# Deeptanshu-sankhwar/horizonml

Measured on AMD Instinct MI355X. Metric: images/sec, higher is better.
Workload: dtype bf16; 1 GPU; model=resnet18_cifar10, global_batch=64, image=3x32x32, parallelism=dp1, optimizer=adam, exec=graph, comm=none

## Files before the change

horizonml_amd/engine/flat.py:

```python
from __future__ import annotations

from typing import List

import torch
import torch.nn as nn

from .. import ops as _ops
from ..models.layers import ConvBNAct, DepthwiseConvBNAct, Linear


class FlatParamManager:
    def __init__(self, model: nn.Module, device: torch.device):
        _ops.extension().set_wgrad_defer(True)
        params = [p for p in model.parameters() if p.requires_grad]
        total = sum(p.numel() for p in params)
        self.params = params
        self.numel = total
        self.master = torch.zeros(total, device=device)
        self.grad = torch.zeros(total, device=device)
        self.shadow = torch.zeros(total, device=device, dtype=torch.bfloat16)
        self.slices = {}
        off = 0
        for p in params:
            n = p.numel()
            with torch.no_grad():
                self.master[off:off + n].copy_(p.data.flatten())
            p.data = self.master[off:off + n].view(p.shape)
            p.grad = self.grad[off:off + n].view(p.shape)
            self.slices[id(p)] = (off, n)
            off += n
        with torch.no_grad():
            self.shadow.copy_(self.master)

        convs = []
        for m in model.modules():
            if isinstance(m, (ConvBNAct, Linear, DepthwiseConvBNAct)):
                woff, wn = self.slices[id(m.weight)]
                m.weight_bf16 = self.shadow[woff:woff + wn].view(
                    m.weight.shape)
                m._managed = True
                if isinstance(m, ConvBNAct):
                    convs.append((m, woff, wn))
        stats_total = sum(2 * m.out_ch for m, _, _ in convs)
        self.stats_arena = torch.zeros(max(1, stats_total), device=device)
        soff = 0
        for m, _, _ in convs:
            m._stats_buf = self.stats_arena[soff:soff + 2 * m.out_ch]
            soff += 2 * m.out_ch

        rsck_total = sum(wn for _, _, wn in convs)
        self.rsck = torch.zeros(rsck_total, device=device,
                                dtype=torch.bfloat16)
        meta: List[List[int]] = []
        doff = 0
        self.max_elem = 1
        for m, woff, wn in convs:
            K, R, S, C = m.weight.shape
            meta.append([woff, doff, wn, (K << 16) | C])
            m._w_rsck = self.rsck[doff:doff + wn].view(R, S, C, K)
            doff += wn
            self.max_elem = max(self.max_elem, wn)
        self.meta = (torch.tensor(meta, dtype=torch.int32, device=device)
                     if meta else None)
        self.refresh_rsck()

    def refresh_rsck(self):
        if self.meta is not None:
            _ops.extension().permute_krsc_rsck(self.shadow, self.rsck,
                                               self.meta, self.max_elem)

    def zero_grad(self):
        self.grad.zero_()


def _sched_buffers(schedule, dev):
    if schedule is None:
        return None, None
    return schedule.table().to(dev), torch.zeros(1, device=dev)


class HorizonAdam:

# ... 122 lines not shown
```

horizonml_amd/models/_functional_gpu.py:

```python
from __future__ import annotations

import torch

from .. import ops as _ops


def _C():
    return _ops.extension()


def _bwd_done(mod):
    cb = getattr(mod, "_bwd_done_cb", None)
    if cb is not None:
        cb()


def _cl(t: torch.Tensor) -> torch.Tensor:
    if t.dim() == 4 and not t.is_contiguous(memory_format=torch.channels_last):
        return t.contiguous(memory_format=torch.channels_last)
    if t.dim() != 4 and not t.is_contiguous():
        return t.contiguous()
    return t


class ConvBNActFn(torch.autograd.Function):
    @staticmethod
    def forward(ctx, x, weight, bn_weight, bn_bias, residual, mod):
        x = _cl(x)
        w_bf16 = mod._shadow()
        if residual is not None:
            residual = _cl(residual)
        stats_buf = (getattr(mod, "_stats_buf", None)
                     if mod.training else None)
        y, convout, smean, sinvstd = _C().conv_bn_act_fwd(
            x, w_bf16, bn_weight, bn_bias, mod.running_mean, mod.running_var,
            mod.stride, mod.padding, mod.momentum, mod.eps, mod.training,
            mod.act, residual, stats_buf)
        ctx.save_for_backward(x, y, convout, w_bf16, bn_weight, bn_bias,
                              smean, sinvstd)
        ctx.mod = mod
        ctx.has_res = residual is not None
        return y

    @staticmethod
    def backward(ctx, dy):
        x, y, convout, w_bf16, gamma, beta, smean, sinvstd = \
            ctx.saved_tensors
        mod = ctx.mod
        need_dx = ctx.needs_input_grad[0]
        w_rsck = getattr(mod, "_w_rsck", None)
        if need_dx and (w_rsck is None or w_rsck.numel() != w_bf16.numel()):
            w_rsck = w_bf16.permute(1, 2, 3, 0).contiguous()
        dy = _cl(dy.to(torch.bfloat16) if dy.dtype != torch.bfloat16 else dy)
        direct = (getattr(mod, "_managed", False)
                  and mod.weight.grad is not None)
        dw_out = mod.weight.grad if direct else None
        dg_out = mod.bn_weight.grad if direct else None
        db_out = mod.bn_bias.grad if direct else None
        dx, dw, dgamma, dbeta, dres = _C().conv_bn_act_bwd(
            dy, y, x, w_bf16, w_rsck if need_dx else w_bf16, convout, gamma,
            beta, smean, sinvstd, mod.stride, mod.padding, mod.act, need_dx,
            ctx.has_res, dw_out, dg_out, db_out, None, None, 0, False, None,
            None)
        _bwd_done(mod)
        if direct:
            return (dx if need_dx else None, None, None, None,
                    dres if ctx.has_res else None, None)
        return (dx if need_dx else None, dw, dgamma, dbeta,
                dres if ctx.has_res else None, None)


def conv_bn_act(x, mod, residual=None):
    return ConvBNActFn.apply(x, mod.weight, mod.bn_weight, mod.bn_bias,
                             residual, mod)


class DwConvBNActFn(torch.autograd.Function):
    @staticmethod
    def forward(ctx, x, weight, bn_weight, bn_bias, residual, mod):
        x = _cl(x)
        w_bf16 = mod._shadow()
        if residual is not None:
            residual = _cl(residual)
        y, convout, smean, sinvstd = _C().dw_conv_bn_fwd(
            x, w_bf16, bn_weight, bn_bias, mod.running_mean,
            mod.running_var, mod.stride, mod.padding, mod.momentum, mod.eps,
            mod.training, mod.act, residual)
        ctx.save_for_backward(x, y, convout, w_bf16, bn_weight, bn_bias,
                              smean, sinvstd)
        ctx.mod = mod
        ctx.has_res = residual is not None
        return y

# ... 86 lines not shown


def linear(x, mod):
    return LinearFn.apply(x, mod.weight, mod.bias, mod)


class CrossEntropyFn(torch.autograd.Function):
    @staticmethod
    def forward(ctx, logits, target, label_smoothing=0.0):
        logits = logits.float().contiguous()
        if label_smoothing == 0.0:
            loss, dlogits = _C().cross_entropy_fwd_bwd(logits, target)
        else:
            loss, dlogits = _C().cross_entropy_ls_fwd_bwd(
                logits, target, float(label_smoothing))
        ctx.save_for_backward(dlogits)
        return loss

    @staticmethod
    def backward(ctx, gout):
        (dlogits,) = ctx.saved_tensors
        return dlogits * gout, None, None


def cross_entropy(logits: torch.Tensor, target: torch.Tensor,
                  label_smoothing: float = 0.0) -> torch.Tensor:
    if logits.is_cuda:
        return CrossEntropyFn.apply(logits, target, float(label_smoothing))
    return torch.nn.functional.cross_entropy(
        logits.float(), target, label_smoothing=float(label_smoothing))


def _rsck(mod, w_bf16):
    w = getattr(mod, "_w_rsck", None)
    if w is None or w.numel() != w_bf16.numel():
        w = w_bf16.permute(1, 2, 3, 0).contiguous()
    return w


class ResBlockFn(torch.autograd.Function):

    @staticmethod
    def forward(ctx, x, mods, ds_mod, *params):
        x = _cl(x)
        training = mods[0].training
        if ds_mod is not None:
            y_ds, convout_ds, smean_ds, sinvstd_ds = _C().conv_bn_act_fwd(
                x, ds_mod._shadow(), ds_mod.bn_weight, ds_mod.bn_bias,
                ds_mod.running_mean, ds_mod.running_var, ds_mod.stride,
                ds_mod.padding, ds_mod.momentum, ds_mod.eps, training,
                ds_mod.act, None,
                getattr(ds_mod, "_stats_buf", None) if training else None)
            identity = y_ds
        else:
            identity = x
        h = x
        saved = [x]
        n = len(mods)
        for i, m in enumerate(mods):
            res = identity if i == n - 1 else None
            y, convout, smean, sinvstd = _C().conv_bn_act_fwd(
                h, m._shadow(), m.bn_weight, m.bn_bias, m.running_mean,
                m.running_var, m.stride, m.padding, m.momentum, m.eps,
                training, m.act, res,
                getattr(m, "_stats_buf", None) if training else None)
            saved += [y, convout, smean, sinvstd, m._shadow(),
# ... 95 lines not shown
```

horizonml_amd/ops/csrc/bind.cpp:

```cpp
#include <torch/extension.h>
#include <c10/hip/HIPStream.h>
#include <c10/hip/HIPCachingAllocator.h>

#include <memory>
#include <vector>

#include "launch.h"

namespace {

using torch::Tensor;

hipStream_t cur_stream() { return c10::hip::getCurrentHIPStream().stream(); }

bool g_deterministic = false;
void set_deterministic(bool on) {
  g_deterministic = on;
  set_kernels_deterministic(on ? 1 : 0);
}
bool deterministic_enabled() { return g_deterministic; }

void set_bn_owner(bool on) { set_kernels_bn_owner(on ? 1 : 0); }
bool bn_owner_enabled() { return kernels_bn_owner() != 0; }
std::vector<int64_t> bn_owner_launches() {
  long f = 0, b = 0;
  bn_owner_launch_counts(&f, &b);
  return {(int64_t)f, (int64_t)b};
}

struct PendingWgrad {
  torch::Tensor x, dconv, dw;
  ConvP p;
};

bool g_wgrad_defer = false;
std::vector<PendingWgrad> g_pending;
torch::Tensor g_wgrad_ws;

void set_wgrad_defer(bool on) { g_wgrad_defer = on; }
bool wgrad_defer_enabled() { return g_wgrad_defer; }
int64_t wgrad_pending() { return (int64_t)g_pending.size(); }

static inline int cdiv_i(long a, long b) { return (int)((a + b - 1) / b); }

void flush_one_group(int lo, int hi);

void flush_wgrad() {
  if (g_pending.empty()) return;
  const int total = (int)g_pending.size();
  int lo = 0;
  while (lo < total) {
    std::vector<const void*> seen;
    int hi = lo;
    for (; hi < total; hi++) {
      const void* ptr = g_pending[hi].dw.data_ptr();
      bool dup = false;
      for (const void* q : seen)
        if (q == ptr) { dup = true; break; }
      if (dup) break;
      seen.push_back(ptr);
    }
// ... 225 lines not shown
                          (int)act, splitk, own, st);
      return {y, convout, smean, sinvstd};
    }
    if (training)
      launch_stats_reduce(ws.data_ptr<float>(), stats_ptr, (long)p.M, K,
                          splitk, st);
    launch_bn_apply_f32(ws.data_ptr<float>(), res_ptr, y.data_ptr(),
                        convout.data_ptr(), stats_ptr,
                        gamma.data_ptr<float>(), beta.data_ptr<float>(),
                        running_mean.data_ptr<float>(),
                        running_var.data_ptr<float>(),
                        training ? smean.data_ptr<float>() : nullptr,
                        training ? sinvstd.data_ptr<float>() : nullptr,
                        (long)p.M, K, (float)momentum, (float)eps,
                        training ? 1 : 0, (int)act, splitk, st);
  } else {
    launch_conv_fwd(x.data_ptr(), w.data_ptr(), convout.data_ptr(),
                    g_deterministic ? nullptr : stats_ptr, p, st);
    if (g_deterministic && training)
      launch_stats_bf16_det(convout.data_ptr(), stats_ptr, (long)p.M, K,
                            st);
    launch_bn_apply(convout.data_ptr(), res_ptr, y.data_ptr(), stats_ptr,
                    gamma.data_ptr<float>(), beta.data_ptr<float>(),
                    running_mean.data_ptr<float>(),
                    running_var.data_ptr<float>(),
                    training ? smean.data_ptr<float>() : nullptr,
                    training ? sinvstd.data_ptr<float>() : nullptr,
                    (long)p.M, K, (float)momentum, (float)eps,
                    training ? 1 : 0, (int)act, st);
  }
  return {y, convout, smean, sinvstd};
}

std::vector<Tensor> conv_bn_act_bwd(
    Tensor dy, Tensor y, Tensor x, Tensor w, Tensor w_rsck, Tensor convout,
    Tensor gamma, Tensor beta, Tensor save_mean, Tensor save_invstd,
    int64_t stride, int64_t pad, int64_t act, bool need_dx, bool has_res,
    c10::optional<Tensor> dw_out, c10::optional<Tensor> dgamma_out,
    c10::optional<Tensor> dbeta_out, c10::optional<Tensor> dx_accum,
    c10::optional<std::vector<Tensor>> fuse_up, int64_t up_mask_mode,
    bool sums_ready, c10::optional<Tensor> sum_dz_in,
    c10::optional<Tensor> sum_dzx_in) {
  check_cl(dy, "dy");
  check_cl(y, "y");
  check_cl(x, "x");
  check_cl(convout, "convout");
  int K = (int)w.size(0), R = (int)w.size(1), S = (int)w.size(2);
  ConvP p = make_convp(x, K, R, S, (int)stride, (int)pad);
  auto fopt = x.options().dtype(torch::kFloat32);
  auto st = cur_stream();

  bool direct = dw_out.has_value();
  int mask_mode = act == 1 ? (has_res ? 1 : 2)
                 : act == 2 ? (has_res ? 3 : 4) : 0;
  Tensor sum_dz, sum_dzx;
  const int own = sums_ready ? 0 : bn_owner_bwd_pick((long)p.M, K, 0);
  if (sums_ready) {
    sum_dz = direct ? *dbeta_out : *sum_dz_in;
    sum_dzx = direct ? *dgamma_out : *sum_dzx_in;
  } else {
    sum_dz = direct ? *dbeta_out : at::zeros({K}, fopt);
    sum_dzx = direct ? *dgamma_out : at::zeros({K}, fopt);
    if (!own)
      launch_bnact_bwd_reduce(dy.data_ptr(), y.data_ptr(),
                              convout.data_ptr(),
                              save_mean.data_ptr<float>(),
                              save_invstd.data_ptr<float>(),
                              gamma.data_ptr<float>(),
// ... 17 lines not shown
                        gamma.data_ptr<float>(), beta.data_ptr<float>(),
                        sum_dz.data_ptr<float>(), sum_dzx.data_ptr<float>(),
                        dconv.data_ptr(), dres_ptr, (long)p.M, K, mask_mode,
                        own, st);
  else
    launch_bn_bwd_apply(dy.data_ptr(), y.data_ptr(), convout.data_ptr(),
                        save_mean.data_ptr<float>(),
                        save_invstd.data_ptr<float>(),
                        gamma.data_ptr<float>(), beta.data_ptr<float>(),
                        sum_dz.data_ptr<float>(), sum_dzx.data_ptr<float>(),
                        dconv.data_ptr(), dres_ptr, (long)p.M, K, mask_mode,
                        st);

  Tensor dw = direct ? *dw_out
                     : at::zeros({(int64_t)K, R, S, (int64_t)p.C}, fopt);
  if (direct && g_wgrad_defer) {
    g_pending.push_back({x, dconv, dw, p});
  } else {
    int msplit = wgrad_msplit(p);
    Tensor ws;
    float* ws_ptr = nullptr;
    if (msplit > 1) {
      ws = at::empty({(long)msplit * K * p.Kd}, fopt);
      ws_ptr = ws.data_ptr<float>();
    }
    launch_wgrad(x.data_ptr(), dconv.data_ptr(), dw.data_ptr<float>(), ws_ptr,
                 p, st);
  }

  TORCH_CHECK(need_dx || !fuse_up.has_value(),
              "fuse_up requires need_dx (the fused reduce rides the dx "
              "production)");
  Tensor dx;
  if (need_dx) {
    TORCH_CHECK(w_rsck.is_contiguous() &&
                    w_rsck.scalar_type() == torch::kBFloat16,
                "w_rsck must be contiguous bf16");
    int accum = dx_accum.has_value() ? 1 : 0;
    dx = accum ? *dx_accum : empty_cl_bf16(p.Nb, p.C, p.H, p.W, x);
    ConvP pd = p;
    pd.M = p.Nb * p.H * p.W;
    pd.Kd = R * S * K;
    int splitk = conv_dgrad_splitk(p);
    const bool fuse = fuse_up.has_value();
    if (splitk > 1) {
      int kchunk = ((pd.Kd + splitk - 1) / splitk + 31) / 32 * 32;
      splitk = (pd.Kd + kchunk - 1) / kchunk;
      Tensor wsd = at::empty({(long)splitk * pd.M * p.C}, fopt);
      launch_conv_dgrad(dconv.data_ptr(), w_rsck.data_ptr(), nullptr,
                        wsd.data_ptr<float>(), splitk, pd, 0, st);
      if (fuse) {
        auto& f = *fuse_up;
        launch_cast_bnact(wsd.data_ptr<float>(), dx.data_ptr(), (long)pd.M,
                          p.C, splitk, accum, f[0].data_ptr(),
                          f[1].defined() ? f[1].data_ptr() : f[0].data_ptr(),
                          f[2].data_ptr<float>(), f[3].data_ptr<float>(),
                          f[4].data_ptr<float>(), f[5].data_ptr<float>(),
                          f[6].data_ptr<float>(), f[7].data_ptr<float>(),
                          (int)up_mask_mode, st);
      } else {
        launch_cast_f32_bf16(wsd.data_ptr<float>(), dx.data_ptr(),
                             (long)pd.M * p.C, splitk, accum, st);
      }
    } else {
      launch_conv_dgrad(dconv.data_ptr(), w_rsck.data_ptr(), dx.data_ptr(),
                        nullptr, 1, pd, accum, st);
      if (fuse) {
        auto& f = *fuse_up;
        launch_bnact_bwd_reduce(dx.data_ptr(), f[1].defined()
                                    ? f[1].data_ptr() : f[0].data_ptr(),
                                f[0].data_ptr(), f[2].data_ptr<float>(),
                                f[3].data_ptr<float>(),
                                f[4].data_ptr<float>(),
                                f[5].data_ptr<float>(),
                                f[6].data_ptr<float>(),
                                f[7].data_ptr<float>(), (long)pd.M, p.C,
                                (int)up_mask_mode, st);
      }
    }
  }
  return {dx, dw, sum_dzx, sum_dz, dres};
}

void check_dw_geometry(int R, int S, int64_t stride, int H, int W,
                       int64_t pad) {
  TORCH_CHECK(R >= 1 && S >= 1 && R * S <= 25,
              "depthwise filter must have R*S <= 25 taps, got ", R, "x", S);
  TORCH_CHECK(stride >= 1, "depthwise stride must be >= 1, got ", stride);
  TORCH_CHECK(pad >= 0, "depthwise pad must be >= 0, got ", pad);
  TORCH_CHECK(H + 2 * pad >= R && W + 2 * pad >= S,
              "depthwise output must be at least 1x1: input ", H, "x", W,
              ", pad ", pad, ", filter ", R, "x", S);
}

std::vector<Tensor> dw_conv_bn_fwd(
    Tensor x, Tensor w, Tensor gamma, Tensor beta, Tensor running_mean,
    Tensor running_var, int64_t stride, int64_t pad, double momentum,
    double eps, bool training, int64_t act, c10::optional<Tensor> residual) {
  check_cl(x, "x");
  TORCH_CHECK(w.is_cuda() && w.scalar_type() == torch::kBFloat16 &&
                  w.is_contiguous() && w.dim() == 3,
              "w must be contiguous bf16 [R,S,C]");
  int Nb = (int)x.size(0), C = (int)x.size(1), H = (int)x.size(2),
      W = (int)x.size(3);
  int R = (int)w.size(0), S = (int)w.size(1);
  TORCH_CHECK((int)w.size(2) == C, "depthwise channel mismatch");
  check_dw_geometry(R, S, stride, H, W, pad);
  int Ho = (H + 2 * (int)pad - R) / (int)stride + 1;
  int Wo = (W + 2 * (int)pad - S) / (int)stride + 1;
  long M = (long)Nb * Ho * Wo;
  auto fopt = x.options().dtype(torch::kFloat32);
  Tensor convout = empty_cl_bf16(Nb, C, Ho, Wo, x);
  Tensor y = empty_cl_bf16(Nb, C, Ho, Wo, x);
// ... 555 lines not shown
        py::arg("wd"), py::arg("decoupled"), py::arg("zero_grad"),
        py::arg("extra_zero") = py::none(), py::arg("grad_bf16") = py::none(),
        py::arg("grad_scale") = 1.0, py::arg("probe_prev") = py::none(),
        py::arg("probe_sumsq") = py::none(),
        py::arg("probe_out") = py::none());
  m.def("sgd_step_sched", &sgd_step_sched, py::arg("master"),
        py::arg("grad"), py::arg("mom"), py::arg("shadow"), py::arg("step_t"),
        py::arg("lr_table"), py::arg("lr_out"), py::arg("lr"), py::arg("mu"),
        py::arg("wd"), py::arg("nesterov"), py::arg("zero_grad"),
        py::arg("grad_bf16") = py::none(), py::arg("grad_scale") = 1.0,
        py::arg("probe_prev") = py::none(),
        py::arg("probe_sumsq") = py::none(),
        py::arg("probe_out") = py::none());
  m.def("permute_krsc_rsck", &permute_krsc_rsck);
  m.def("grad_divergence", &grad_divergence);
  m.def("normalize_u8", &normalize_u8);
  m.def("augment_normalize_u8", &augment_normalize_u8, py::arg("x"),
        py::arg("state"), py::arg("mean"), py::arg("std"), py::arg("pad"),
        py::arg("flip"), py::arg("params") = py::none());
  m.def("bn_reduce_bench", &bn_reduce_bench);
  m.def("bn_fwd_pair_bench", &bn_fwd_pair_bench);
  m.def("bn_bwd_pair_bench", &bn_bwd_pair_bench);
  m.def("set_bn_owner", &set_bn_owner);
  m.def("bn_owner_enabled", &bn_owner_enabled);
  m.def("bn_owner_launches", &bn_owner_launches);
  m.def("set_deterministic", &set_deterministic);
  m.def("deterministic_enabled", &deterministic_enabled);
  m.def("set_wgrad_defer", &set_wgrad_defer);
  m.def("wgrad_defer_enabled", &wgrad_defer_enabled);
  m.def("wgrad_pending", &wgrad_pending);
  m.def("flush_wgrad", &flush_wgrad);
  m.def("flush_wgrad_range", &flush_wgrad_range);
  m.def("wgrad_only", &wgrad_only);
}
```

horizonml_amd/ops/csrc/conv_kernels.hip:

```cpp
#include "common.h"

template <int MODE>
DEV int a_addr(const ConvP& p, const MagicP& mg, int m, int k, bool& valid) {
  if (MODE == 0) {
    valid = (m < p.M) & (k < p.Kd);
    return m * p.Kd + k;
  } else if (MODE == 1) {
    unsigned n = fdiv(m, mg, 0), hw = fmod(m, n, mg, 0);
    unsigned ho = fdiv(hw, mg, 1), wo = fmod(hw, ho, mg, 1);
    unsigned r = fdiv(k, mg, 2), rm = fmod(k, r, mg, 2);
    unsigned sx = fdiv(rm, mg, 3), c = fmod(rm, sx, mg, 3);
    int hi = (int)ho * p.str - p.pad + (int)r;
    int wi = (int)wo * p.str - p.pad + (int)sx;
    valid = (m < p.M) & (k < p.Kd) & (hi >= 0) & (hi < p.H) & (wi >= 0) & (wi < p.W);
    return (((int)n * p.H + hi) * p.W + wi) * p.C + (int)c;
  } else {
    unsigned n = fdiv(m, mg, 0), hw = fmod(m, n, mg, 0);
    unsigned hi = fdiv(hw, mg, 1), wi = fmod(hw, hi, mg, 1);
    unsigned r = fdiv(k, mg, 2), rm = fmod(k, r, mg, 2);
    unsigned sx = fdiv(rm, mg, 3), ko = fmod(rm, sx, mg, 3);
    int hs = (int)hi + p.pad - (int)r, ws = (int)wi + p.pad - (int)sx;
    bool ok = (m < p.M) & (k < p.Kd) & (hs >= 0) & (ws >= 0) &&
              (hs % p.str == 0) && (ws % p.str == 0);
    int ho = hs / p.str, wo = ws / p.str;
// ... 48 lines not shown
          ++hi;
        }
      }
    }
  } else {
    for (int e = 0; e < 8; e++) {
      bool ok;
      int a = a_addr<MODE>(p, mg, m, k + e, ok);
      v.e[e] = ok ? src[a] : (bf16)0.f;
    }
  }
  return v;
}

template <int MODE, bool VEC>
DEV V8 load8_b(const bf16* __restrict__ src, const ConvP& p,
               const MagicP& mg, int n, int k, int Ntot) {
  V8 v;
  if (VEC) {
    bool ok;
    int a = b_addr<MODE>(p, mg, n, k, Ntot, ok);
    if (ok) v.u = *(const uint4*)(src + a);
    else v.u = uint4{0, 0, 0, 0};
  } else {
    for (int e = 0; e < 8; e++) {
      bool ok;
      int a = b_addr<MODE>(p, mg, n, k + e, Ntot, ok);
      v.e[e] = ok ? src[a] : (bf16)0.f;
    }
  }
  return v;
}

#define LDA 40

template <int MODE, bool VECA, bool VECB, bool STATS, bool SPLIT,
          int TM = 64, int TN = 64>
__global__ __launch_bounds__(256) void k_conv_mfma(
    const bf16* __restrict__ A, const bf16* __restrict__ Bw,
    bf16* __restrict__ Y, float* __restrict__ ws_out,
    float* __restrict__ stats, ConvP p, MagicP mg, int Ntot, int kchunk,
    int accum) {
  constexpr int AC = TM / 64;
  constexpr int BC = TN / 64;
  constexpr int MI = TM / 32;
  constexpr int NI = TN / 32;
  constexpr int WM = TM / 2, WN = TN / 2;
  __shared__ bf16 As[2][TM * LDA];
  __shared__ bf16 Bs[2][TN * LDA];

  const int m0 = blockIdx.y * TM, n0 = blockIdx.x * TN;
  const int kbeg = SPLIT ? blockIdx.z * kchunk : 0;
  const int kend = SPLIT ? min(p.Kd, kbeg + kchunk) : p.Kd;
  const int tid = threadIdx.x;
  const int srow = tid >> 2, scol = (tid & 3) * 8;
  const int lane = tid & 63, wave = tid >> 6;
  const int wr = wave >> 1, wc = wave & 1;
  const int fr = lane & 15, fk = lane >> 4;

  f32x4 acc[MI][NI] = {};

#pragma unroll
  for (int j = 0; j < AC; j++) {
    V8 a0 = load8_a<MODE, VECA>(A, p, mg, m0 + j * 64 + srow, kbeg + scol);
    *(V8*)&As[0][(j * 64 + srow) * LDA + scol] = a0;
  }
#pragma unroll
  for (int j = 0; j < BC; j++) {
    V8 b0 = load8_b<MODE, VECB>(Bw, p, mg, n0 + j * 64 + srow, kbeg + scol,
                                Ntot);
    *(V8*)&Bs[0][(j * 64 + srow) * LDA + scol] = b0;
  }
  V8 a_nx[AC], b_nx[BC];
  if (kbeg + 32 < kend) {
#pragma unroll
    for (int j = 0; j < AC; j++)
      a_nx[j] = load8_a<MODE, VECA>(A, p, mg, m0 + j * 64 + srow,
                                    kbeg + 32 + scol);
#pragma unroll
    for (int j = 0; j < BC; j++)
      b_nx[j] = load8_b<MODE, VECB>(Bw, p, mg, n0 + j * 64 + srow,
                                    kbeg + 32 + scol, Ntot);
  }
  __syncthreads();

  int buf = 0;
  for (int k0 = kbeg; k0 < kend; k0 += 32) {
    if (k0 + 32 < kend) {
#pragma unroll
      for (int j = 0; j < AC; j++)
        *(V8*)&As[buf ^ 1][(j * 64 + srow) * LDA + scol] = a_nx[j];
#pragma unroll
      for (int j = 0; j < BC; j++)
        *(V8*)&Bs[buf ^ 1][(j * 64 + srow) * LDA + scol] = b_nx[j];
      if (k0 + 64 < kend) {
#pragma unroll
        for (int j = 0; j < AC; j++)
          a_nx[j] = load8_a<MODE, VECA>(A, p, mg, m0 + j * 64 + srow,
                                        k0 + 64 + scol);
#pragma unroll
        for (int j = 0; j < BC; j++)
          b_nx[j] = load8_b<MODE, VECB>(Bw, p, mg, n0 + j * 64 + srow,
                                        k0 + 64 + scol, Ntot);
      }
    }
    bf16x8 af[MI], bf[NI];
#pragma unroll
    for (int mi = 0; mi < MI; mi++)
      af[mi] =
          *(const bf16x8*)&As[buf][(wr * WM + mi * 16 + fr) * LDA + fk * 8];
#pragma unroll
    for (int ni = 0; ni < NI; ni++)
      bf[ni] =
          *(const bf16x8*)&Bs[buf][(wc * WN + ni * 16 + fr) * LDA + fk * 8];
#pragma unroll
    for (int mi = 0; mi < MI; mi++)
#pragma unroll
      for (int ni = 0; ni < NI; ni++)
        acc[mi][ni] = __builtin_amdgcn_mfma_f32_16x16x32_bf16(
            af[mi], bf[ni], acc[mi][ni], 0, 0, 0);
    buf ^= 1;
    __syncthreads();
  }

  float ssum[NI], ssq[NI];
#pragma unroll
  for (int ni = 0; ni < NI; ni++) ssum[ni] = ssq[ni] = 0.f;
#pragma unroll
  for (int mi = 0; mi < MI; mi++) {
#pragma unroll
    for (int ni = 0; ni < NI; ni++) {
      int gn = n0 + wc * WN + ni * 16 + fr;
#pragma unroll
      for (int q = 0; q < 4; q++) {
        int gm = m0 + wr * WM + mi * 16 + fk * 4 + q;
        if (gm < p.M && gn < Ntot) {
          float v = acc[mi][ni][q];
          if (SPLIT) {
            ws_out[(long)blockIdx.z * p.M * Ntot + (long)gm * Ntot + gn] = v;
          } else {
            long yi = (long)gm * Ntot + gn;
            if (accum) v += b2f(Y[yi]);
            Y[yi] = f2b(v);
            if (STATS) {
              ssum[ni] += v;
              ssq[ni] += v * v;
            }
// ... 487 lines not shown
    if (vec && s) CASE_T(true, true, true, TM, TN);                    \
    else if (vec) CASE_T(true, true, false, TM, TN);                   \
    else if (s) CASE_T(false, false, true, TM, TN);                    \
    else CASE_T(false, false, false, TM, TN);                          \
  } while (0)
  if (tile == 3) DISPATCH(256, 64);
  else if (tile == 2) DISPATCH(128, 128);
  else if (tile == 1) DISPATCH(128, 64);
  else DISPATCH(64, 64);
#undef DISPATCH
#undef CASE_T
}

extern "C" void launch_conv_fwd_splitk(const void* x, const void* w,
                                       float* ws, ConvP p, int splitk,
                                       hipStream_t st) {
  int kchunk = cdiv_h(cdiv_h(p.Kd, splitk), 32) * 32;
  splitk = cdiv_h(p.Kd, kchunk);
  bool vec = (p.C % 8) == 0 && (p.Kd % 8) == 0;
  auto A = (const bf16*)x;
  auto B = (const bf16*)w;
  MagicP mg = make_magic(p, 1);
  int tile = pick_tile(p.M, p.K);
#define SK_T(VA, VB, TM, TN)                                              k_conv_mfma<1, VA, VB, false, true, TM, TN><<<grid, 256, 0, st>>>(          A, B, nullptr, ws, nullptr, p, mg, p.K, kchunk, 0)
#define DISPATCH(TM, TN)                                                  do {                                                                      dim3 grid(cdiv_h(p.K, TN), cdiv_h(p.M, TM), splitk);                    if (vec) SK_T(true, true, TM, TN);                                      else SK_T(false, false, TM, TN);                                      } while (0)
  if (tile == 3) DISPATCH(256, 64);
  else if (tile == 2) DISPATCH(128, 128);
  else if (tile == 1) DISPATCH(128, 64);
  else DISPATCH(64, 64);
#undef DISPATCH
#undef SK_T
}

extern "C" void launch_conv_dgrad(const void* dz, const void* w_rsck,
                                  void* dx, float* ws, int splitk, ConvP p,
                                  int accum, hipStream_t st) {
  bool vec = (p.K % 8) == 0;
  auto A = (const bf16*)dz;
  auto B = (const bf16*)w_rsck;
  if (splitk > 1) {
    int kchunk = cdiv_h(cdiv_h(p.Kd, splitk), 32) * 32;
    splitk = cdiv_h(p.Kd, kchunk);
    MagicP mg = make_magic(p, 2);
    int tile = pick_tile_dgrad(p.M, p.C);
#define SKD_T(VA, VB, TM, TN)                                             k_conv_mfma<2, VA, VB, false, true, TM, TN><<<grid, 256, 0, st>>>(          A, B, nullptr, ws, nullptr, p, mg, p.C, kchunk, 0)
#define DISPATCH(TM, TN)                                                  do {                                                                      dim3 grid(cdiv_h(p.C, TN), cdiv_h(p.M, TM), splitk);                    if (vec) SKD_T(true, true, TM, TN);                                     else SKD_T(false, false, TM, TN);                                     } while (0)
    if (tile == 3) DISPATCH(256, 64);
    else if (tile == 2) DISPATCH(128, 128);
    else if (tile == 1) DISPATCH(128, 64);
    else DISPATCH(64, 64);
#undef DISPATCH
#undef SKD_T
  } else {
    MagicP mg = make_magic(p, 2);
    int tile = pick_tile_dgrad(p.M, p.C);
#define DGRAD_T(VA, VB, TM, TN)                                         \
  k_conv_mfma<2, VA, VB, false, false, TM, TN><<<grid, 256, 0, st>>>(   \
      A, B, (bf16*)dx, nullptr, nullptr, p, mg, p.C, 0, accum)
#define DISPATCH(TM, TN)                                                \
  do {                                                                  \
    dim3 grid(cdiv_h(p.C, TN), cdiv_h(p.M, TM));                        \
    if (vec) DGRAD_T(true, true, TM, TN);                               \
    else DGRAD_T(false, false, TM, TN);                                 \
  } while (0)
    if (tile == 3) DISPATCH(256, 64);
    else if (tile == 2) DISPATCH(128, 128);
    else if (tile == 1) DISPATCH(128, 64);
    else DISPATCH(64, 64);
#undef DISPATCH
#undef DGRAD_T
  }
}
// ... 66 lines not shown
```

horizonml_amd/ops/csrc/launch.h:

```cpp
#pragma once
#include <hip/hip_runtime_api.h>

#include <cstdlib>
#include <type_traits>

struct ConvP {
  int Nb, H, W, C, K;
  int Ho, Wo, R, S;
  int str, pad;
  int M, Kd;
};

struct MagicP {
  unsigned m[4];
  int s[4];
  unsigned d[4];
};

constexpr int WG_MAX_TASKS = 20;

struct WgradTask {
  const void* X;
  const void* Dz;
  float* out;
  ConvP p;
  MagicP mg;
  int Ntot, mchunk, msplit, tx, ty;
  int base;
  int vec;
};

struct WgradBatchArgs {
  int n;
  WgradTask t[WG_MAX_TASKS];
};

struct WredTask {
  const float* ws;
  float* dW;
  long n;
  int msplit;
  int base;
};

struct WredBatchArgs {
  int n;
  WredTask t[WG_MAX_TASKS];
};

static_assert(sizeof(WgradBatchArgs) <= 4096 && sizeof(WredBatchArgs) <= 4096,
              "batched wgrad task tables must fit the kernarg segment");
static_assert(std::is_trivially_copyable_v<WgradBatchArgs> &&
                  std::is_trivially_copyable_v<WredBatchArgs>,
              "batched wgrad task tables are copied into the kernarg segment");

inline void magic_u32(unsigned d, unsigned* m, int* sh) {
  if (d <= 1) { *m = 0; *sh = 0; return; }
  int p = 0;
  while ((1ull << p) < d) p++;
  *m = (unsigned)((((unsigned long long)((1ull << p) - d) << 32) / d) + 1);
  *sh = p;
}

inline MagicP make_magic(const ConvP& p, int mode) {
  MagicP mg{};
  unsigned d[4];
  if (mode == 2) {
    d[0] = (unsigned)(p.H * p.W);
    d[1] = (unsigned)p.W;
    d[2] = (unsigned)(p.S * p.K);
    d[3] = (unsigned)p.K;
  } else {
    d[0] = (unsigned)(p.Ho * p.Wo);
    d[1] = (unsigned)p.Wo;
    d[2] = (unsigned)(p.S * p.C);
    d[3] = (unsigned)p.C;
  }
  for (int i = 0; i < 4; i++) {
    mg.d[i] = d[i] ? d[i] : 1;
    magic_u32(mg.d[i], &mg.m[i], &mg.s[i]);
  }
  return mg;
}

inline long env_long(const char* name, long dflt) {
  const char* e = getenv(name);
  return e ? atol(e) : dflt;
}

extern "C" {

int conv_fwd_splitk(ConvP p);
int conv_dgrad_splitk(ConvP p);
void launch_conv_fwd(const void* x, const void* w, void* y, float* stats,
                     ConvP p, hipStream_t st);
void launch_conv_fwd_splitk(const void* x, const void* w, float* ws, ConvP p,
                            int splitk, hipStream_t st);
void launch_conv_dgrad(const void* dz, const void* w_rsck, void* dx,
                       float* ws, int splitk, ConvP p, int accum,
                       hipStream_t st);
void launch_gemm_bf16(const void* a, const void* b, void* c, int M, int N,
                      int K, hipStream_t st);
int wgrad_msplit(ConvP p);
void launch_wgrad(const void* x, const void* dz, float* dw, float* ws,
                  ConvP p, hipStream_t st);
void launch_wgrad_batched_t(const WgradBatchArgs* args, int blocks, int tk3,
                            int tko, hipStream_t st);
void launch_wgrad_reduce_batched(const WredBatchArgs* args, int blocks,
                                 hipStream_t st);

void set_kernels_deterministic(int on);
void set_kernels_bn_owner(int on);
int kernels_bn_owner();
void bn_owner_launch_counts(long* fwd, long* bwd);
int bn_owner_fwd_pick(long M, int C, int lpr_req);
int bn_owner_bwd_pick(long M, int C, int lpr_req);

void launch_bn_apply(const void* x, const void* res, void* y,
                     const float* stats, const float* gamma,
                     const float* beta, float* rmean, float* rvar,
                     float* smean, float* sinvstd, long M, int C,
                     float momentum, float eps, int training, int act,
                     hipStream_t st);
void launch_bn_apply_f32(const float* ws, const void* res, void* y,
                         void* convout, const float* stats,
                         const float* gamma, const float* beta, float* rmean,
                         float* rvar, float* smean, float* sinvstd, long M,
                         int C, float momentum, float eps, int training,
                         int act, int nsplit, hipStream_t st);
void launch_stats_reduce(const float* ws, float* stats, long M, int C,
                         int nsplit, hipStream_t st);
void launch_stats_bf16_det(const void* x, float* stats, long M, int C,
// ... 100 lines not shown
```

Baseline: 64130 images/sec.

## Read KRSC weights directly in dgrad via LDS transpose reads, drop RSCK copy

Adds a KRSC variant of the MFMA dgrad kernel that loads weights in their native KRSC layout, stores them into LDS with a swizzled offset, and uses ds_read_tr16 transpose reads to build the B fragments. This removes the per-step permute_krsc_rsck kernel after each optimizer step and the separate RSCK weight buffer. It is enabled by default through HZ_DGRAD_KRSC. The dgrad main loop now does strided global loads along K plus transpose LDS reads, which could be slower than the old contiguous loads.

```diff
diff --git a/horizonml_amd/engine/flat.py b/horizonml_amd/engine/flat.py
--- a/horizonml_amd/engine/flat.py
+++ b/horizonml_amd/engine/flat.py
@@ -48,6 +48,14 @@
             m._stats_buf = self.stats_arena[soff:soff + 2 * m.out_ch]
             soff += 2 * m.out_ch
 
+        self.meta = None
+        self.max_elem = 1
+        if _ops.extension().dgrad_krsc_enabled():
+            self.rsck = torch.zeros(0, device=device, dtype=torch.bfloat16)
+            for m, _, _ in convs:
+                if hasattr(m, "_w_rsck"):
+                    del m._w_rsck
+            return
         rsck_total = sum(wn for _, _, wn in convs)
         self.rsck = torch.zeros(rsck_total, device=device,
                                 dtype=torch.bfloat16)
diff --git a/horizonml_amd/models/_functional_gpu.py b/horizonml_amd/models/_functional_gpu.py
--- a/horizonml_amd/models/_functional_gpu.py
+++ b/horizonml_amd/models/_functional_gpu.py
@@ -48,9 +48,7 @@
             ctx.saved_tensors
         mod = ctx.mod
         need_dx = ctx.needs_input_grad[0]
-        w_rsck = getattr(mod, "_w_rsck", None)
-        if need_dx and (w_rsck is None or w_rsck.numel() != w_bf16.numel()):
-            w_rsck = w_bf16.permute(1, 2, 3, 0).contiguous()
+        w_rsck = _rsck(mod, w_bf16) if need_dx else None
         dy = _cl(dy.to(torch.bfloat16) if dy.dtype != torch.bfloat16 else dy)
         direct = (getattr(mod, "_managed", False)
                   and mod.weight.grad is not None)
@@ -58,7 +56,7 @@
         dg_out = mod.bn_weight.grad if direct else None
         db_out = mod.bn_bias.grad if direct else None
         dx, dw, dgamma, dbeta, dres = _C().conv_bn_act_bwd(
-            dy, y, x, w_bf16, w_rsck if need_dx else w_bf16, convout, gamma,
+            dy, y, x, w_bf16, w_rsck, convout, gamma,
             beta, smean, sinvstd, mod.stride, mod.padding, mod.act, need_dx,
             ctx.has_res, dw_out, dg_out, db_out, None, None, 0, False, None,
             None)
@@ -211,6 +209,8 @@
 
 
 def _rsck(mod, w_bf16):
+    if _C().dgrad_krsc_enabled():
+        return None
     w = getattr(mod, "_w_rsck", None)
     if w is None or w.numel() != w_bf16.numel():
         w = w_bf16.permute(1, 2, 3, 0).contiguous()
diff --git a/horizonml_amd/ops/csrc/bind.cpp b/horizonml_amd/ops/csrc/bind.cpp
--- a/horizonml_amd/ops/csrc/bind.cpp
+++ b/horizonml_amd/ops/csrc/bind.cpp
@@ -27,6 +27,10 @@
   bn_owner_launch_counts(&f, &b);
   return {(int64_t)f, (int64_t)b};
 }
+
+bool g_dgrad_krsc = env_long("HZ_DGRAD_KRSC", 1) != 0;
+void set_dgrad_krsc(bool on) { g_dgrad_krsc = on; }
+bool dgrad_krsc_enabled() { return g_dgrad_krsc; }
 
 struct PendingWgrad {
   torch::Tensor x, dconv, dw;
@@ -318,8 +322,101 @@
   return {y, convout, smean, sinvstd};
 }
 
+Tensor dgrad_dx(const Tensor& dconv, const Tensor& w,
+                const c10::optional<Tensor>& w_rsck, const ConvP& p,
+                const c10::optional<Tensor>& dx_accum,
+                const c10::optional<std::vector<Tensor>>& fuse_up,
+                int up_mask_mode, hipStream_t st) {
+  const bool krsc =
+      !w_rsck.has_value() || w_rsck->data_ptr() == w.data_ptr();
+  const Tensor& wt = krsc ? w : *w_rsck;
+  TORCH_CHECK(wt.is_contiguous() && wt.scalar_type() == torch::kBFloat16,
+              krsc ? "w must be contiguous bf16"
+                   : "w_rsck must be contiguous bf16");
+  TORCH_CHECK(wt.numel() == (int64_t)p.K * p.R * p.S * p.C,
+              "dgrad weight has ", wt.numel(), " elements, expected K*R*S*C");
+  auto fopt = dconv.options().dtype(torch::kFloat32);
+  const int layout = krsc ? DGRAD_W_KRSC : DGRAD_W_RSCK;
+  int accum = dx_accum.has_value() ? 1 : 0;
+  Tensor dx = accum ? *dx_accum : empty_cl_bf16(p.Nb, p.C, p.H, p.W, dconv);
+  ConvP pd = p;
+  pd.M = p.Nb * p.H * p.W;
+  pd.Kd = p.R * p.S * p.K;
+  int splitk = conv_dgrad_splitk(p);
+  const bool fuse = fuse_up.has_value();
+  if (splitk > 1) {
+    int kchunk = ((pd.Kd + splitk - 1) / splitk + 31) / 32 * 32;
+    splitk = (pd.Kd + kchunk - 1) / kchunk;
+    Tensor wsd = at::empty({(long)splitk * pd.M * p.C}, fopt);
+    launch_conv_dgrad(dconv.data_ptr(), wt.data_ptr(), nullptr,
+                      wsd.data_ptr<float>(), splitk, pd, 0, layout, st);
+    if (fuse) {
+      auto& f = *fuse_up;
+      launch_cast_bnact(wsd.data_ptr<float>(), dx.data_ptr(), (long)pd.M,
+                        p.C, splitk, accum, f[0].data_ptr(),
+                        f[1].defined() ? f[1].data_ptr() : f[0].data_ptr(),
+                        f[2].data_ptr<float>(), f[3].data_ptr<float>(),
+                        f[4].data_ptr<float>(), f[5].data_ptr<float>(),
+                        f[6].data_ptr<float>(), f[7].data_ptr<float>(),
+                        up_mask_mode, st);
+    } else {
+      launch_cast_f32_bf16(wsd.data_ptr<float>(), dx.data_ptr(),
+                           (long)pd.M * p.C, splitk, accum, st);
+    }
+  } else {
+    launch_conv_dgrad(dconv.data_ptr(), wt.data_ptr(), dx.data_ptr(), nullptr,
+                      1, pd, accum, layout, st);
+    if (fuse) {
+      auto& f = *fuse_up;
+      launch_bnact_bwd_reduce(dx.data_ptr(), f[1].defined()
+                                  ? f[1].data_ptr() : f[0].data_ptr(),
+                              f[0].data_ptr(), f[2].data_ptr<float>(),
+                              f[3].data_ptr<float>(),
+                              f[4].data_ptr<float>(),
+                              f[5].data_ptr<float>(),
+                              f[6].data_ptr<float>(),
+                              f[7].data_ptr<float>(), (long)pd.M, p.C,
+                              up_mask_mode, st);
+    }
+  }
+  return dx;
+}
+
+Tensor conv_dgrad_only(Tensor dz, Tensor w, int64_t H, int64_t W,
+                       int64_t stride, int64_t pad,
+                       c10::optional<Tensor> w_rsck,
+                       c10::optional<Tensor> dx_accum) {
+  check_cl(dz, "dz");
+  TORCH_CHECK(w.dim() == 4 && w.size(0) == dz.size(1),
+              "w must be [K,R,S,C] with K = dz channels");
+  ConvP p{};
+  p.Nb = (int)dz.size(0);
+  p.C = (int)w.size(3);
+  p.H = (int)H;
+  p.W = (int)W;
+  p.K = (int)w.size(0);
+  p.R = (int)w.size(1);
+  p.S = (int)w.size(2);
+  p.str = (int)stride;
+  p.pad = (int)pad;
+  p.Ho = (p.H + 2 * p.pad - p.R) / p.str + 1;
+  p.Wo = (p.W + 2 * p.pad - p.S) / p.str + 1;
+  p.M = p.Nb * p.Ho * p.Wo;
+  p.Kd = p.R * p.S * p.C;
+  TORCH_CHECK(dz.size(2) == p.Ho && dz.size(3) == p.Wo,
+              "dz spatial size does not match H, W, stride, pad");
+  if (dx_accum.has_value()) {
+    check_cl(*dx_accum, "dx_accum");
+    TORCH_CHECK(dx_accum->size(0) == p.Nb && dx_accum->size(1) == p.C &&
+                    dx_accum->size(2) == p.H && dx_accum->size(3) == p.W,
+                "dx_accum must be [Nb,C,H,W]");
+  }
+  return dgrad_dx(dz, w, w_rsck, p, dx_accum, c10::nullopt, 0, cur_stream());
+}
+
 std::vector<Tensor> conv_bn_act_bwd(
-    Tensor dy, Tensor y, Tensor x, Tensor w, Tensor w_rsck, Tensor convout,
+    Tensor dy, Tensor y, Tensor x, Tensor w, c10::optional<Tensor> w_rsck,
+    Tensor convout,
     Tensor gamma, Tensor beta, Tensor save_mean, Tensor save_invstd,
     int64_t stride, int64_t pad, int64_t act, bool need_dx, bool has_res,
     c10::optional<Tensor> dw_out, c10::optional<Tensor> dgamma_out,
@@ -403,53 +500,9 @@
               "fuse_up requires need_dx (the fused reduce rides the dx "
               "production)");
   Tensor dx;
-  if (need_dx) {
-    TORCH_CHECK(w_rsck.is_contiguous() &&
-                    w_rsck.scalar_type() == torch::kBFloat16,
-                "w_rsck must be contiguous bf16");
-    int accum = dx_accum.has_value() ? 1 : 0;
-    dx = accum ? *dx_accum : empty_cl_bf16(p.Nb, p.C, p.H, p.W, x);
-    ConvP pd = p;
-    pd.M = p.Nb * p.H * p.W;
-    pd.Kd = R * S * K;
-    int splitk = conv_dgrad_splitk(p);
-    const bool fuse = fuse_up.has_value();
-    if (splitk > 1) {
-      int kchunk = ((pd.Kd + splitk - 1) / splitk + 31) / 32 * 32;
-      splitk = (pd.Kd + kchunk - 1) / kchunk;
-      Tensor wsd = at::empty({(long)splitk * pd.M * p.C}, fopt);
-      launch_conv_dgrad(dconv.data_ptr(), w_rsck.data_ptr(), nullptr,
-                        wsd.data_ptr<float>(), splitk, pd, 0, st);
-      if (fuse) {
-        auto& f = *fuse_up;
-        launch_cast_bnact(wsd.data_ptr<float>(), dx.data_ptr(), (long)pd.M,
-                          p.C, splitk, accum, f[0].data_ptr(),
-                          f[1].defined() ? f[1].data_ptr() : f[0].data_ptr(),
-                          f[2].data_ptr<float>(), f[3].data_ptr<float>(),
-                          f[4].data_ptr<float>(), f[5].data_ptr<float>(),
-                          f[6].data_ptr<float>(), f[7].data_ptr<float>(),
-                          (int)up_mask_mode, st);
-      } else {
-        launch_cast_f32_bf16(wsd.data_ptr<float>(), dx.data_ptr(),
-                             (long)pd.M * p.C, splitk, accum, st);
-      }
-    } else {
-      launch_conv_dgrad(dconv.data_ptr(), w_rsck.data_ptr(), dx.data_ptr(),
-                        nullptr, 1, pd, accum, st);
-      if (fuse) {
-        auto& f = *fuse_up;
-        launch_bnact_bwd_reduce(dx.data_ptr(), f[1].defined()
-                                    ? f[1].data_ptr() : f[0].data_ptr(),
-                                f[0].data_ptr(), f[2].data_ptr<float>(),
-                                f[3].data_ptr<float>(),
-                                f[4].data_ptr<float>(),
-                                f[5].data_ptr<float>(),
-                                f[6].data_ptr<float>(),
-                                f[7].data_ptr<float>(), (long)pd.M, p.C,
-                                (int)up_mask_mode, st);
-      }
-    }
-  }
+  if (need_dx)
+    dx = dgrad_dx(dconv, w, w_rsck, p, dx_accum, fuse_up, (int)up_mask_mode,
+                  st);
   return {dx, dw, sum_dzx, sum_dz, dres};
 }
 
@@ -1071,4 +1124,7 @@
   m.def("flush_wgrad", &flush_wgrad);
   m.def("flush_wgrad_range", &flush_wgrad_range);
   m.def("wgrad_only", &wgrad_only);
-}
+  m.def("conv_dgrad_only", &conv_dgrad_only);
+  m.def("set_dgrad_krsc", &set_dgrad_krsc);
+  m.def("dgrad_krsc_enabled", &dgrad_krsc_enabled);
+}
diff --git a/horizonml_amd/ops/csrc/conv_kernels.hip b/horizonml_amd/ops/csrc/conv_kernels.hip
--- a/horizonml_amd/ops/csrc/conv_kernels.hip
+++ b/horizonml_amd/ops/csrc/conv_kernels.hip
@@ -104,10 +104,41 @@
   return v;
 }
 
+template <int TN>
+DEV int krsc_off(int k, int n) {
+  const int f = TN == 64 ? (((k >> 1) & 1) | (((k >> 3) & 1) << 1))
+                         : ((k & 3) | (((k >> 3) & 1) << 2));
+  return k * TN + ((((n >> 4) ^ f)) << 4) + (n & 15);
+}
+
+template <bool VEC>
+DEV V8 load8_b_krsc(const bf16* __restrict__ src, const ConvP& p,
+                    const MagicP& mg, int n, int k, int kend, int Ntot) {
+  V8 v;
+  unsigned rs = fdiv(k, mg, 3), ko = fmod(k, rs, mg, 3);
+  const bool kok = k < kend;
+  const int a = ((int)ko * p.R * p.S + (int)rs) * p.C + n;
+  if (VEC) {
+    if (kok && n < Ntot) v.u = *(const uint4*)(src + a);
+    else v.u = uint4{0, 0, 0, 0};
+  } else {
+    for (int e = 0; e < 8; e++)
+      v.e[e] = (kok && n + e < Ntot) ? src[a + e] : (bf16)0.f;
+  }
+  return v;
+}
+
+typedef __attribute__((ext_vector_type(4))) __bf16 bf16x4;
+typedef __attribute__((address_space(3))) bf16x4 lds_bf16x4;
+
+DEV bf16x4 lds_read_tr16(const bf16* sp) {
+  return __builtin_amdgcn_ds_read_tr16_b64_v4bf16((lds_bf16x4*)sp);
+}
+
 #define LDA 40
 
 template <int MODE, bool VECA, bool VECB, bool STATS, bool SPLIT,
-          int TM = 64, int TN = 64>
+          int TM = 64, int TN = 64, bool KRSC = false>
 __global__ __launch_bounds__(256) void k_conv_mfma(
     const bf16* __restrict__ A, const bf16* __restrict__ Bw,
     bf16* __restrict__ Y, float* __restrict__ ws_out,
@@ -118,8 +149,10 @@
   constexpr int MI = TM / 32;
   constexpr int NI = TN / 32;
   constexpr int WM = TM / 2, WN = TN / 2;
-  __shared__ bf16 As[2][TM * LDA];
-  __shared__ bf16 Bs[2][TN * LDA];
+  static_assert(!KRSC || MODE == 2, "KRSC is a dgrad B layout");
+  static_assert(!KRSC || TN == 64 || TN == 128, "krsc_off covers TN 64/128");
+  __shared__ __attribute__((aligned(16))) bf16 As[2][TM * LDA];
+  __shared__ __attribute__((aligned(16))) bf16 Bs[2][TN * LDA];
 
   const int m0 = blockIdx.y * TM, n0 = blockIdx.x * TN;
   const int kbeg = SPLIT ? blockIdx.z * kchunk : 0;
@@ -129,6 +162,27 @@
   const int lane = tid & 63, wave = tid >> 6;
   const int wr = wave >> 1, wc = wave & 1;
   const int fr = lane & 15, fk = lane >> 4;
+  const int bkrow = tid / (TN / 8), bncol = (tid % (TN / 8)) * 8;
+  constexpr int BKSTEP = 256 / (TN / 8);
+
+  auto load_b = [&](int j, int kt) -> V8 {
+    if (KRSC)
+      return load8_b_krsc<VECB>(Bw, p, mg, n0 + bncol,
+                                kt + j * BKSTEP + bkrow, kend, Ntot);
+    return load8_b<MODE, VECB>(Bw, p, mg, n0 + j * 64 + srow, kt + scol,
+                               Ntot);
+  };
+  auto store_b = [&](int b, int j, const V8& v) {
+    if (KRSC)
+      *(V8*)&Bs[b][krsc_off<TN>(j * BKSTEP + bkrow, bncol)] = v;
+    else
+      *(V8*)&Bs[b][(j * 64 + srow) * LDA + scol] = v;
+  };
+  int boff[NI];
+#pragma unroll
+  for (int ni = 0; ni < NI; ni++)
+    boff[ni] = krsc_off<TN>(fk * 8 + (fr >> 2),
+                            wc * WN + ni * 16 + (fr & 3) * 4);
 
   f32x4 acc[MI][NI] = {};
 
@@ -138,11 +192,7 @@
     *(V8*)&As[0][(j * 64 + srow) * LDA + scol] = a0;
   }
 #pragma unroll
-  for (int j = 0; j < BC; j++) {
-    V8 b0 = load8_b<MODE, VECB>(Bw, p, mg, n0 + j * 64 + srow, kbeg + scol,
-                                Ntot);
-    *(V8*)&Bs[0][(j * 64 + srow) * LDA + scol] = b0;
-  }
+  for (int j = 0; j < BC; j++) store_b(0, j, load_b(j, kbeg));
   V8 a_nx[AC], b_nx[BC];
   if (kbeg + 32 < kend) {
 #pragma unroll
@@ -150,9 +200,7 @@
       a_nx[j] = load8_a<MODE, VECA>(A, p, mg, m0 + j * 64 + srow,
                                     kbeg + 32 + scol);
 #pragma unroll
-    for (int j = 0; j < BC; j++)
-      b_nx[j] = load8_b<MODE, VECB>(Bw, p, mg, n0 + j * 64 + srow,
-                                    kbeg + 32 + scol, Ntot);
+    for (int j = 0; j < BC; j++) b_nx[j] = load_b(j, kbeg + 32);
   }
   __syncthreads();
 
@@ -163,17 +211,14 @@
       for (int j = 0; j < AC; j++)
         *(V8*)&As[buf ^ 1][(j * 64 + srow) * LDA + scol] = a_nx[j];
 #pragma unroll
-      for (int j = 0; j < BC; j++)
-        *(V8*)&Bs[buf ^ 1][(j * 64 + srow) * LDA + scol] = b_nx[j];
+      for (int j = 0; j < BC; j++) store_b(buf ^ 1, j, b_nx[j]);
       if (k0 + 64 < kend) {
 #pragma unroll
         for (int j = 0; j < AC; j++)
           a_nx[j] = load8_a<MODE, VECA>(A, p, mg, m0 + j * 64 + srow,
                                         k0 + 64 + scol);
 #pragma unroll
-        for (int j = 0; j < BC; j++)
-          b_nx[j] = load8_b<MODE, VECB>(Bw, p, mg, n0 + j * 64 + srow,
-                                        k0 + 64 + scol, Ntot);
+        for (int j = 0; j < BC; j++) b_nx[j] = load_b(j, k0 + 64);
       }
     }
     bf16x8 af[MI], bf[NI];
@@ -182,9 +227,16 @@
       af[mi] =
           *(const bf16x8*)&As[buf][(wr * WM + mi * 16 + fr) * LDA + fk * 8];
 #pragma unroll
-    for (int ni = 0; ni < NI; ni++)
-      bf[ni] =
-          *(const bf16x8*)&Bs[buf][(wc * WN + ni * 16 + fr) * LDA + fk * 8];
+    for (int ni = 0; ni < NI; ni++) {
+      if (KRSC) {
+        bf16x4 lo = lds_read_tr16(&Bs[buf][boff[ni]]);
+        bf16x4 hi = lds_read_tr16(&Bs[buf][boff[ni] + 4 * TN]);
+        bf[ni] = __builtin_shufflevector(lo, hi, 0, 1, 2, 3, 4, 5, 6, 7);
+      } else {
+        bf[ni] =
+            *(const bf16x8*)&Bs[buf][(wc * WN + ni * 16 + fr) * LDA + fk * 8];
+      }
+    }
 #pragma unroll
     for (int mi = 0; mi < MI; mi++)
 #pragma unroll
@@ -738,12 +790,55 @@
 #undef SK_T
 }
 
-extern "C" void launch_conv_dgrad(const void* dz, const void* w_rsck,
-                                  void* dx, float* ws, int splitk, ConvP p,
-                                  int accum, hipStream_t st) {
+template <int TM, int TN>
+static void dgrad_krsc_t(const bf16* A, const bf16* B, bf16* dx, float* ws,
+                         bool split, int splitk, int kchunk, const ConvP& p,
+                         const MagicP& mg, int accum, hipStream_t st) {
+  dim3 grid(cdiv_h(p.C, TN), cdiv_h(p.M, TM), split ? splitk : 1);
+  const bool va = (p.K % 8) == 0, vb = (p.C % 8) == 0;
+#define KRSC_T(VA, VB)                                                      \
+  do {                                                                      \
+    if (split)                                                              \
+      k_conv_mfma<2, VA, VB, false, true, TM, TN, true>                     \
+          <<<grid, 256, 0, st>>>(A, B, nullptr, ws, nullptr, p, mg, p.C,    \
+                                 kchunk, 0);                                \
+    else                                                                    \
+      k_conv_mfma<2, VA, VB, false, false, TM, TN, true>                    \
+          <<<grid, 256, 0, st>>>(A, B, dx, nullptr, nullptr, p, mg, p.C, 0, \
+                                 accum);                                    \
+  } while (0)
+  if (va && vb) KRSC_T(true, true);
+  else if (va) KRSC_T(true, false);
+  else if (vb) KRSC_T(false, true);
+  else KRSC_T(false, false);
+#undef KRSC_T
+}
+
+extern "C" void launch_conv_dgrad(const void* dz, const void* w, void* dx,
+                                  float* ws, int splitk, ConvP p, int accum,
+                                  int w_layout, hipStream_t st) {
   bool vec = (p.K % 8) == 0;
   auto A = (const bf16*)dz;
-  auto B = (const bf16*)w_rsck;
+  auto B = (const bf16*)w;
+  if (w_layout == DGRAD_W_KRSC) {
+    const bool split = splitk > 1;
+    int kchunk = 0;
+    if (split) {
+      kchunk = cdiv_h(cdiv_h(p.Kd, splitk), 32) * 32;
+      splitk = cdiv_h(p.Kd, kchunk);
+    }
+    MagicP mg = make_magic(p, 2);
+    int tile = pick_tile_dgrad(p.M, p.C);
+#define DISPATCH(TM, TN)                                                  \
+  dgrad_krsc_t<TM, TN>(A, B, (bf16*)dx, ws, split, splitk, kchunk, p, mg, \
+                       accum, st)
+    if (tile == 3) DISPATCH(256, 64);
+    else if (tile == 2) DISPATCH(128, 128);
+    else if (tile == 1) DISPATCH(128, 64);
+    else DISPATCH(64, 64);
+#undef DISPATCH
+    return;
+  }
   if (splitk > 1) {
     int kchunk = cdiv_h(cdiv_h(p.Kd, splitk), 32) * 32;
     splitk = cdiv_h(p.Kd, kchunk);
diff --git a/horizonml_amd/ops/csrc/launch.h b/horizonml_amd/ops/csrc/launch.h
--- a/horizonml_amd/ops/csrc/launch.h
+++ b/horizonml_amd/ops/csrc/launch.h
@@ -53,6 +53,8 @@
 static_assert(std::is_trivially_copyable_v<WgradBatchArgs> &&
                   std::is_trivially_copyable_v<WredBatchArgs>,
               "batched wgrad task tables are copied into the kernarg segment");
+
+enum DgradWLayout { DGRAD_W_RSCK = 0, DGRAD_W_KRSC = 1 };
 
 inline void magic_u32(unsigned d, unsigned* m, int* sh) {
   if (d <= 1) { *m = 0; *sh = 0; return; }
@@ -96,8 +98,8 @@
                      ConvP p, hipStream_t st);
 void launch_conv_fwd_splitk(const void* x, const void* w, float* ws, ConvP p,
                             int splitk, hipStream_t st);
-void launch_conv_dgrad(const void* dz, const void* w_rsck, void* dx,
-                       float* ws, int splitk, ConvP p, int accum,
+void launch_conv_dgrad(const void* dz, const void* w, void* dx, float* ws,
+                       int splitk, ConvP p, int accum, int w_layout,
                        hipStream_t st);
 void launch_gemm_bf16(const void* a, const void* b, void* c, int M, int N,
                       int K, hipStream_t st);
```

New measurement: 66700 images/sec, median of 6. 4.0% higher.
